# m-dayani/EORB_SLAM

Measured on AMD Instinct MI355X. Metric: front-end frames/s (event-accumulate + extract + match) per GPU; HBM GB/s vs roofline, higher is better.
Workload: dtype f32; 1 GPU; BASELINE.json configs[1]: synthetic 1000000 events/slice on 240x180 (shapes generator, DAVIS sensor pixels; raw (x,y,t,p) records resolved on the GPU through the calibrator's undistortion maps built from the EvETHZ intrinsics, as the reference loader does on the CPU), ev2im_gauss sigma=1 -> ORB-1000 (1.2, 4 levels, FAST 10/0, edge 19) -> SearchForInitialization vs previous slice; input=raw, sequences_per_gpu=1, parallelism=1 GPU

## Files before the change

eorb_slam_amd/csrc/eorb_fe.hip:

```cpp
#include "eorb_ctx.h"
#include "match_args.h"
#include "project_args.h"
#include "kfdb.h"
#include "twoview.h"
#include "sim3.h"
#include "mlpnp.h"
#include "newpts.h"
#include <stdarg.h>
#include <stdio.h>
#include <string.h>
#include <algorithm>
#include <functional>
#include <vector>

namespace eorb {

int set_err(eorb_ctx* c, int code, const char* fmt, ...)
{
    char buf[512];
    va_list ap; va_start(ap, fmt); vsnprintf(buf, sizeof(buf), fmt, ap); va_end(ap);
    if (c) c->err = buf;
    return code;
}

// ... 346 lines not shown
}

long long eorb_debug_counter(eorb_ctx* c, const char* name)
{
    if (!c || !name) return -1;
    if (!strcmp(name, "slot_calls")) return c->sl_calls;
    if (!strcmp(name, "accum_route")) return c->accum_route;
    if (!strcmp(name, "slot_rank_ok")) return c->sl_rank_ok;
    if (!strcmp(name, "dict_hits")) return c->pd_hits;
    if (!strcmp(name, "dict_misses")) return c->pd_misses;
    if (!strcmp(name, "dict_positions")) return c->pd_valid ? c->pd_K : 0;
    if (!strcmp(name, "slot_scatter_form")) return c->sl_last_rank;
    if (!strcmp(name, "slot_chunk")) return c->sl_last_chunk;
    if (!strcmp(name, "slot_binning")) return c->sl_last_binning;
    if (!strcmp(name, "kfdb_slot_cap")) return c->kfdb.slot_cap;
    if (!strcmp(name, "kfdb_word_cap")) return c->kfdb.word_cap;
    if (!strcmp(name, "slot_parts")) return c->sl_last_parts;
    if (!strcmp(name, "slot_hot_overflow")) {
        long long n = 0;
        for (int part = 0; part < std::max(c->sl_last_parts, 1); part++) {
            if (!c->sl_ws[part].hot.p) continue;
            uint32_t h = 0;
            if (hipMemcpyAsync(&h, (uint32_t*)c->sl_ws[part].hot.p + 33, sizeof(h), hipMemcpyDeviceToHost, c->stream) != hipSuccess || hipStreamSynchronize(c->stream) != hipSuccess) return -1;
            n += h;
        }
        return n;
    }
    if (!strcmp(name, "oct_lds_only")) return c->orb.oct_all_lds[0] | (c->orb.oct_all_lds[1] << 1);
    if (!strcmp(name, "oct_lds_bytes")) return c->orb.oct_lds[0];
    if (!strcmp(name, "oct_dynamic")) return c->orb.oct_dyn[0] != 0 ? 1 : 0;
    if (!strcmp(name, "oct_redo_levels")) {
        const int nl = c->orb.nlevels;
        if (!c->orb.oct_dyn[0] || !c->lvl_cnt.p || nl <= 0) return 0;
        std::vector<int32_t> f((size_t)nl);
        if (hipMemcpyAsync(f.data(), (const char*)c->lvl_cnt.p + (size_t)nl * sizeof(int32_t) + 64, sizeof(int32_t) * (size_t)nl, hipMemcpyDeviceToHost, c->stream) != hipSuccess ||
            hipStreamSynchronize(c->stream) != hipSuccess) return -1;
        long long r = 0; for (int v : f) r += v ? 1 : 0;
        return r;
    }
    if (!strcmp(name, "oct_direct_cap")) return c->orb.oct_direct_cap[0] | ((long long)c->orb.oct_direct_cap[1] << 16);
    if (!strcmp(name, "oct_scratch_bytes")) return c->orb.oct_scratch[0];
    if (!strcmp(name, "slot_hot_items")) {
        long long n = 0;
        for (int part = 0; part < std::max(c->sl_last_parts, 1); part++) {
            if (!c->sl_ws[part].hot.p) continue;
            uint32_t h[16];
// ... 3597 lines not shown
```

eorb_slam_amd/csrc/ev_plan.h:

```cpp
#pragma once
#include <math.h>
#include <stddef.h>
#include <stdint.h>
#include <algorithm>

namespace eorb {

constexpr int kTile = 8;
constexpr int kChunk = 4096;
constexpr int kScatWaves = 8;
constexpr int kSlotScatWaves = 8;
constexpr int kSlotCountWaves = 16;
constexpr int kHotCap = 8192;
constexpr int kHotRows = 240;
constexpr int kDdLog = 20;
constexpr int kDirectSlices = 8;
constexpr int64_t kDirectMaxEvents = 16384;

struct AccumShape {
    int h;
    int R, dup;
    int TX, TY, NT, NTp;
    int nbits;
    int64_t nev, per_slice;
};
inline AccumShape accum_shape(int W, int H, float sigma, int mode_count, int B, int64_t nev)
{
    AccumShape S;
    S.h = mode_count ? 0 : (int)ceil((double)sigma * 3.0);
    S.R = (2 * S.h <= kTile) ? ((S.h == 0) ? 1 : 2) : 3;
    S.dup = S.R * S.R;
    S.TX = (W + kTile - 1) / kTile; S.TY = (H + kTile - 1) / kTile; S.NT = S.TX * S.TY; S.NTp = (S.NT + 1) & ~1;
    S.nbits = 1; while ((1 << S.nbits) < S.NT) S.nbits++;
    S.nev = nev; S.per_slice = B > 0 ? nev / B : 0;
    return S;
}
// ... 135 lines not shown
inline int slot_binning_code(const SlotBinPlan& p) { return p.count | p.record << 2 | p.scatter << 4; }

inline bool plan_slot_binning(const AccumShape& S, int stride_in, int64_t nsrc, int dict, const SlotScatterChoice& sc, const AccumKnobs& K, SlotBinPlan* out)
{
    const int stride = dict ? (dict == 2 ? 2 : -4) : stride_in;
    const size_t lds_c = 4 * (((size_t)nsrc + 2) / 2) + (size_t)kSlotCountWaves * S.NTp * 2;
    const bool lds_fits = S.TX <= 127 && S.TY <= 127 && lds_c <= 159 * 1024;
    const size_t lds_p = plan_slot_lds_pre(S.NT, sc.chunk);
    const bool pre_fits = K.slot_prerank && sc.rank && lds_p <= 158 * 1024;
    const int scat = sc.rank ? kScatRank : kScatBallot;
    SlotBinPlan p{kCountLds, kRecAsIs, scat, stride, stride, lds_c, sc.lds};
    if (dict) {
        if (!lds_fits) return false;
        p.count = kCountLdsKeyed;
        if (pre_fits && dict == 2) { p.record = kRecRanked8; p.scatter = kScatPre; p.lds_scatter = lds_p; }
    }
    else if (!lds_fits) { p.count = kCountGlobal; p.lds_count = sizeof(uint32_t) * (size_t)S.NT; }
    else if (pre_fits && (stride == 16 || stride == 4 || stride == 2) && nsrc <= 65535) { p.record = kRecRanked8; p.scatter = kScatPre; p.lds_scatter = lds_p; }
    else if (stride == 16 && nsrc <= 65535 && sc.rank) { p.record = kRecShort2; p.scat_stride = 2; }
    *out = p;
    return true;
}

struct SlotGatherPlan {
    size_t lds; int wg_per_cu, nw, rounds, Gt, max_per_tile;
    uint32_t prio_ref, hot_min, hot_cap; int hot_waves;
};
inline SlotGatherPlan plan_slot_gather(const AccumShape& S, int B, int64_t nev, int nparts, int sl_null, int ncu, const AccumKnobs& K)
{
    SlotGatherPlan g;
    g.lds = (size_t)(sl_null + 1) * 256;
    g.wg_per_cu = std::max(1, (int)((160 * 1024) / g.lds));
    g.nw = std::min(16, std::max(1, 16 / g.wg_per_cu));
    if (K.slot_waves >= 1 && K.slot_waves <= 16) g.nw = K.slot_waves;
    g.nw = std::min(g.nw, std::max(1, B));
    g.rounds = K.slot_rounds >= 1 ? K.slot_rounds : 4;
    g.Gt = S.NT + g.rounds * ncu * g.wg_per_cu;
    g.max_per_tile = (B + g.nw - 1) / g.nw;
    g.prio_ref = (uint32_t)std::min<int64_t>(std::max<int64_t>(4096, nev / 2000), 0x7fffffff);
    g.hot_min = sl_null <= kHotRows ? (uint32_t)std::min<int64_t>(std::max<int64_t>(4096, nev * nparts / 16000), 0x7fffffff) : 0u;
    const long long hot_over = K.slot_hot_min;
    if (hot_over >= 0) g.hot_min = (sl_null <= kHotRows && hot_over > 0) ? (uint32_t)std::min<long long>(std::max<long long>(hot_over, 64), 0x7fffffff) : 0u;
    g.hot_cap = K.slot_hot_cap > 0 ? (uint32_t)std::min(K.slot_hot_cap, kHotCap) : (uint32_t)kHotCap;
    g.hot_waves = K.slot_hot_waves > 0 ? K.slot_hot_waves : 8 * ncu;
    return g;
}

inline int plan_first_route(const AccumShape& S, AccumRequest Q, const AccumKnobs& K, const DictState& D, int W, int H, float sigma, bool rank_ok,
                            bool slots_usable = true)
{
    SlotScatterChoice sc;
    int set = Q.raw ? kSetMaps : kSetNone, wide = 0;
    if (plan_bulk_eligible(S, Q, K) && plan_bulk_fits(S, K)) {
        if (plan_dict_usable(S, Q, K, D, W, H, sigma) && plan_slot_shape(S, Q.B, K, rank_ok, &sc)) return kFormSlots | kSetDict;
        Q.raw = 2; set = kSetPerCall;
    }
    else if (plan_direct(S, Q, K)) return kFormDirect | set;
    if (plan_slot_eligible(S, Q, K) && slots_usable && plan_slot_shape(S, Q.B, K, rank_ok, &sc)) return kFormSlots | set;
    if (Q.raw == 3 || Q.raw == 4) {
        Q.raw = 1; wide = kRouteWidened;
        if (plan_direct(S, Q, K)) return kFormDirect | set | wide;
    }
    return kFormLists | set | (plan_sparse_gather(S, Q, K) ? kRouteSparse : 0) | wide;
}

}
```

eorb_slam_amd/csrc/ev_slots.hip:

```cpp
#include "eorb_ctx.h"
#include "ev_common.h"
#include "dev_math.h"
#include "sl_hot_asm.h"
#include <algorithm>
#include <stdlib.h>
#include <string.h>
#include <vector>

namespace eorb {

constexpr uint32_t kNoSlot = 0xffu;
typedef uint16_t slot_entry;
constexpr uint32_t kEntryTag = 0x1000u;
constexpr uint16_t kNoGeo = 0xffffu;

__global__ void sl_assign_kernel(const uint32_t* __restrict__ src_info, int nsrc, int W, int H, int h, int TX,
                                 uint32_t* __restrict__ tile_nslots, uint2* __restrict__ slot_tab, uint16_t* __restrict__ slot_geo,
                                 int* __restrict__ info)
{
    const int i = blockIdx.x * blockDim.x + threadIdx.x;
    if (i >= nsrc) { if (i == nsrc) slot_geo[i] = kNoGeo; return; }
    const uint32_t w = src_info[i];
    const int xi = (int)(int16_t)(w & 0xffff), yi = (int)(int16_t)(w >> 16);
    uint2 o = make_uint2(0u, 0xffffffffu);
// ... 678 lines not shown
        const bool act = ((h >> 3) & 7u) != 0u;
        uint32_t r = 0xffffffffu;
        noise[(threadIdx.x * 33 + t) & 1023] = h;
        uint32_t rr[4];
#pragma unroll
        for (int q = 0; q < 4; q++) {
            rr[q] = 0xffffffffu;
            if (act && ((h >> (12 + q)) & 1u)) { const uint32_t o = atomicAdd(&cnt[a >> 1], 1u << (16 * (a & 1))); rr[q] = (o >> (16 * (a & 1))) & 0xffffu; }
        }
#pragma unroll
        for (int q = 0; q < 4; q++) {
            r = rr[q];
            for (int j = 0; j < 64; j++) {
                const uint32_t aj = __shfl(a, j, 64), rj = __shfl(r, j, 64);
                if (r != 0xffffffffu && rj != 0xffffffffu && j < lane && aj == a && !(rj < r)) nbad++;
            }
        }
        __syncthreads();
    }
    if (noise[threadIdx.x] == 0x12345u) nbad += 0;
    if (nbad) atomicAdd(bad, nbad);
}

constexpr int kHotBuckets = 16;
static_assert(kHotRows == SL_HOT_NROWS, "plan_slot_gather (ev_plan.h) and sl_hot_kernel's register rows");
struct HotDesc { uint32_t slice, tile, cnt, off_lo, off_hi, tx0, ty0, rows_off; };
__global__ __launch_bounds__(256) void sl_plan_kernel(const uint32_t* __restrict__ tile_cnt, const uint32_t* __restrict__ tile_base,
                                                      const int64_t* __restrict__ slice_ebase, int B, int NT, int TX, uint32_t hot_min,
                                                      const uint32_t* __restrict__ nslots, const uint32_t* __restrict__ rowbase,
                                                      uint4* __restrict__ items, uint32_t* __restrict__ tile_w, uint32_t* __restrict__ tile_m,
                                                      uint32_t* __restrict__ ctr, uint32_t* __restrict__ hot_cnt, HotDesc* __restrict__ hot_items,
                                                      uint32_t hot_cap )
{
    extern __shared__ uint32_t pc[];
    __shared__ uint32_t red[8];
    __shared__ uint32_t hb[kHotBuckets], hbase[kHotBuckets];
    uint32_t* hloc = pc + B;
    const int t = blockIdx.x, tid = threadIdx.x;
    const bool hot_ok = hot_min != 0u && nslots[t] <= (uint32_t)SL_HOT_NROWS;
    if (tid < kHotBuckets) hb[tid] = 0u;
    __syncthreads();
    for (int s = tid; s < B; s += blockDim.x) {
        const uint32_t c = tile_cnt[(size_t)s * NT + t];
        uint32_t v = c;
        if (hot_ok && c >= hot_min) {
            const int lg = 31 - __clz(c), lg0 = 31 - __clz(hot_min);
            const int q = (lg - lg0) * 4 + (int)((c >> max(lg - 2, 0)) & 3u) - (int)((hot_min >> max(lg0 - 2, 0)) & 3u);
            const int b = kHotBuckets - 1 - min(max(q, 0), kHotBuckets - 1);
            hloc[s] = ((uint32_t)b << 16) | atomicAdd(&hb[b], 1u);
            v = c | 0x80000000u;
        }
        pc[s] = v;
    }
    __syncthreads();
    if (tid < kHotBuckets) hbase[tid] = hb[tid] ? atomicAdd(&hot_cnt[tid], hb[tid]) : 0u;
    __syncthreads();
    uint32_t sum = 0, mx = 0;
    for (int s = tid; s < B; s += blockDim.x) {
        uint32_t v = pc[s];
        if (v & 0x80000000u) {
            const uint32_t c = v & 0x7fffffffu, b = hloc[s] >> 16, k = hbase[b] + (hloc[s] & 0xffffu);
            if (k < hot_cap) {
                const uint64_t off = ((uint64_t)slice_ebase[s] + tile_base[(size_t)s * NT + t]) * sizeof(slot_entry);
                HotDesc d; d.slice = (uint32_t)s; d.tile = (uint32_t)t; d.cnt = c; d.off_lo = (uint32_t)off; d.off_hi = (uint32_t)(off >> 32);
                d.tx0 = (uint32_t)(t % TX) * 8u; d.ty0 = (uint32_t)(t / TX) * 8u; d.rows_off = rowbase[t] * 256u;
                hot_items[(size_t)b * kHotCap + k] = d;
            } else { v = c; pc[s] = v; atomicAdd(&hot_cnt[33], 1u); }
        }
        if (!(v & 0x80000000u)) { sum += v; mx = max(mx, v); }
    }
    __syncthreads();
    const bool sorted = B <= 2048;
    for (int s = tid; s < B; s += blockDim.x) {
        const uint32_t c = pc[s];
        int rank = s;
        if (sorted) { rank = 0; for (int j = 0; j < B; j++) { const uint32_t v = pc[j]; rank += (v > c || (v == c && j < s)) ? 1 : 0; } }
        const uint64_t off = ((uint64_t)slice_ebase[s] + tile_base[(size_t)s * NT + t]) * sizeof(slot_entry);
        items[(size_t)t * B + rank] = make_uint4((uint32_t)s | (c & 0x80000000u), c & 0x7fffffffu, (uint32_t)off, (uint32_t)(off >> 32));
    }
#pragma unroll
    for (int d = 32; d >= 1; d >>= 1) { sum += (uint32_t)__shfl_xor((int)sum, d, 64); mx = max(mx, (uint32_t)__shfl_xor((int)mx, d, 64)); }
    if ((tid & 63) == 0) { red[tid >> 6] = sum; red[4 + (tid >> 6)] = mx; }
    __syncthreads();
    if (tid == 0) {
        tile_w[t] = red[0] + red[1] + red[2] + red[3];
        tile_m[t] = max(max(red[4], red[5]), max(red[6], red[7]));
        ctr[t] = 0u;
    }
}
__global__ __launch_bounds__(1024) void sl_tasks_kernel(const uint32_t* __restrict__ tile_w, const uint32_t* __restrict__ tile_m, int NT, int G,
                                                        int max_per_tile, uint32_t* __restrict__ scratch , uint32_t* __restrict__ task_tile, uint32_t* __restrict__ hot_cnt,
                                                        uint32_t hot_cap)
{
    if (threadIdx.x < kHotBuckets) hot_cnt[threadIdx.x] = min(hot_cnt[threadIdx.x], hot_cap);
    __shared__ unsigned long long wred[16];
    __shared__ uint32_t wsum[16], wsum2[16];
    const int tid = threadIdx.x, lane = tid & 63, wave = tid >> 6;
    unsigned long long tot = 0;
    for (int t = tid; t < NT; t += 1024) tot += tile_w[t];
#pragma unroll
    for (int d = 32; d >= 1; d >>= 1) tot += (unsigned long long)__shfl_xor((long long)tot, d, 64);
    if (lane == 0) wred[wave] = tot;
    __syncthreads();
    tot = 0;
    for (int w = 0; w < 16; w++) tot += wred[w];
    const unsigned long long spare = (unsigned long long)max(G - NT, 0);
    uint32_t* nsorted = scratch; uint32_t* tsorted = scratch + NT;
    extern __shared__ uint32_t tm[];
    for (int t = tid; t < NT; t += 1024) tm[t] = tile_m[t];
    __syncthreads();
    for (int t = tid; t < NT; t += 1024) {
        const uint32_t m = tm[t];
        int rank = 0;
        for (int u = 0; u < NT; u++) { const uint32_t v = tm[u]; rank += (v > m || (v == m && u < t)) ? 1 : 0; }
        uint32_t n = 1u + (tot ? (uint32_t)((unsigned long long)tile_w[t] * spare / tot) : 0u);
        n = min(n, (uint32_t)max(max_per_tile, 1));
        nsorted[rank] = n; tsorted[rank] = (uint32_t)t;
// ... 423 lines not shown
                                                               L.d_tile_base, p.d_entries());
        }
        else if (L.nchunks && bp.scatter == kScatRank) {
            const SlScatRankFn fn = sl_scatter_rank_fn(bp.scat_stride, waves);
            if ((rc = sl_optin(c, (const void*)fn, 159 * 1024))) return rc;
            fn<<<L.nchunks, 64 * waves, bp.lds_scatter, p.M>>>(d_ev, L.d_chunks, p.d_tab(), T.w, T.h, p.TX, p.NT, chunk, L.d_slice_eb, L.d_segbase, L.d_tile_base, p.d_entries());
        }
        else if (L.nchunks)
            sl_scatter_kernel<<<L.nchunks, 64 * kSlotScatWaves, bp.lds_scatter, p.M>>>(d_ev, L.d_chunks, p.d_tab(), bp.scat_stride, T.w, T.h, p.TX, p.TY, p.NT, chunk, L.d_slice_eb, L.d_segbase,
                                                                                         L.d_tile_base, p.d_entries());
        EORB_LAUNCH_CHECK(c, "ev_bin (slot) kernels");
    }
    EORB_HIP(c, hipEventRecord(p.E[2], p.M));
    return EORB_OK;
}

static int slots_fork_plan(const SlotPart& p)
{
    eorb_ctx* c = p.c; const BinLayout& L = p.L; const SlotGatherPlan& g = p.gp;
    EORB_HIP(c, hipEventRecord(p.E[0], p.M));
    EORB_HIP(c, hipStreamWaitEvent(p.P, p.E[0], 0));
    EORB_HIP(c, hipMemsetAsync(p.ws.hot.p, 0, 256, p.P));
    sl_plan_kernel<<<p.NT, 256, sizeof(uint32_t) * 2 * (size_t)p.B, p.P>>>(L.d_tile_cnt, L.d_tile_base, L.d_slice_eb, p.B, p.NT, p.TX, g.hot_min, p.d_nslots(), p.d_rowbase(),
                                                                             p.d_items(), p.d_tile_w(), p.d_tile_m(), p.d_ctr(), p.d_hot_cnt(), p.d_hot_items(), g.hot_cap);
    sl_tasks_kernel<<<1, 1024, sizeof(uint32_t) * (size_t)p.NT, p.P>>>(p.d_tile_w(), p.d_tile_m(), p.NT, g.Gt, g.max_per_tile, p.d_scr(), p.d_task(), p.d_hot_cnt(), g.hot_cap);
    EORB_HIP(c, hipEventRecord(p.E[1], p.P));
    return EORB_OK;
}

static int slots_gather(const SlotPart& p)
{
    eorb_ctx* c = p.c; const PosTables& T = p.T; const SlotGatherPlan& g = p.gp;
    int rc;
    SlotGather Pg{p.d_task(), p.d_items(), (const uint8_t*)p.ws.entries.p, p.d_nslots(), p.d_rowbase(), (const float*)T.sl_rows.p,
                  p.d_tile_w(), p.d_ctr(), p.d_f32, p.d_minmax_enc, p.d_info(), (int*)c->status.p, p.B, p.W, p.H, p.TX, p.NT, T.sl_null, g.prio_ref, nullptr};
#ifdef EORB_SLOT_TRACE
    EORB_HIP(c, hipMemsetAsync(c->sl_trace.p, 0, sizeof(unsigned long long) * 6 * 16 * (size_t)g.Gt + 64, p.M));
    Pg.trace = (unsigned long long*)c->sl_trace.p + 8;
    c->sl_trace_n = (long long)g.Gt * 16;
#endif
    if ((rc = sl_optin(c, (const void*)sl_gather_kernel, 160 * 1024))) return rc;
    if (g.hot_min) {
        EORB_HIP(c, hipStreamWaitEvent(p.Hs, p.E[2], 0));
        EORB_HIP(c, hipStreamWaitEvent(p.Hs, p.E[1], 0));
        sl_hot_kernel<<<g.hot_waves, 64, 0, p.Hs>>>(p.d_hot_cnt(), p.d_hot_cnt() + 32, p.d_hot_items(), kHotCap, (const float*)T.sl_rows.p, p.d_entries(), p.d_f32, p.d_minmax_enc, p.W, p.H);
    }
    EORB_HIP(c, hipEventRecord(p.E[3], p.Hs));
    if (p.G != p.M) EORB_HIP(c, hipStreamWaitEvent(p.G, p.E[2], 0));
    EORB_HIP(c, hipStreamWaitEvent(p.G, p.E[1], 0));
    {
        ProfScope ps(c, "ev_gather", p.G);
        sl_gather_kernel<<<g.Gt, 64 * g.nw, g.lds, p.G>>>(Pg);
    }
    EORB_HIP(c, hipEventRecord(p.E[4], p.G));
    EORB_LAUNCH_CHECK(c, "sl_gather_kernel");
    return EORB_OK;
}

int ev_slots_accumulate(eorb_ctx* c, const PosTables& T, const AccumShape& S, const void* d_events, int stride, const int64_t* h_offsets, int B, int W, int H,
                        float* d_f32, uint32_t* d_minmax_enc, const SlotDict* dict)
{
    const AccumKnobs K = accum_knobs(c);
    const int nparts = (K.slot_halves > 0 && B >= 2) ? 2 : 1;
    SlotScatterChoice sc;
    if (!plan_slot_shape(S, B, K, c->sl_rank_ok == 1, &sc)) return kSlotDeclined;
    for (int b = 0; b < B; b++) {
        const int64_t s = h_offsets[b], e = h_offsets[b + 1];
        if (e < s) return set_err(c, EORB_E_ARG, "ev_accumulate: offsets not monotone");
// ... 35 lines not shown
```

eorb_slam_amd/csrc/sl_hot_asm.h:

```cpp
#define SL_HOT_NROWS 240
#define SL_HOT_ASM \
    "s_setprio 3\n" \
    "v_mbcnt_lo_u32_b32 v242, -1, 0\n" \
    "v_mbcnt_hi_u32_b32 v242, -1, v242\n" \
    "v_and_b32 v249, 1, v242\n" \
    "v_lshlrev_b32 v249, 7, v249\n" \
    "v_lshlrev_b32 v252, 6, v242\n" \
    "v_and_b32 v243, 7, v242\n" \
    "v_lshrrev_b32 v244, 3, v242\n" \
    "v_lshlrev_b32 v242, 2, v242\n" \
    "v_mov_b32 v246, v243\n" \
    "v_mov_b32 v247, v244\n" \
    "s_load_dwordx16 s[36:51], %[hcnt], 0x0\n" \
    "s_waitcnt lgkmcnt(0)\n" \
    "SLH_ITEM:\n" \
    "v_mov_b32 v245, 1\n" \
    "v_mov_b32 v248, 0\n" \
    "s_mov_b64 s[62:63], exec\n" \
    "s_mov_b64 exec, 1\n" \
    "global_atomic_add v245, v248, v245, %[ticket] sc0\n" \
    "s_waitcnt vmcnt(0)\n" \
    "s_mov_b64 exec, s[62:63]\n" \
    "s_nop 0\n" \
    "v_readfirstlane_b32 s60, v245\n" \
    "s_mov_b32 s61, 0\n" \
    "s_cmp_lt_u32 s60, s36\n" \
    "s_cbranch_scc1 SLH_FOUND\n" \
    "s_sub_u32 s60, s60, s36\n" \
    "s_add_u32 s61, s61, 1\n" \
    "s_cmp_lt_u32 s60, s37\n" \
    "s_cbranch_scc1 SLH_FOUND\n" \
    "s_sub_u32 s60, s60, s37\n" \
    "s_add_u32 s61, s61, 1\n" \
    "s_cmp_lt_u32 s60, s38\n" \
    "s_cbranch_scc1 SLH_FOUND\n" \
    "s_sub_u32 s60, s60, s38\n" \
    "s_add_u32 s61, s61, 1\n" \
    "s_cmp_lt_u32 s60, s39\n" \
    "s_cbranch_scc1 SLH_FOUND\n" \
    "s_sub_u32 s60, s60, s39\n" \
    "s_add_u32 s61, s61, 1\n" \
    "s_cmp_lt_u32 s60, s40\n" \
    "s_cbranch_scc1 SLH_FOUND\n" \
    "s_sub_u32 s60, s60, s40\n" \
    "s_add_u32 s61, s61, 1\n" \
    "s_cmp_lt_u32 s60, s41\n" \
    "s_cbranch_scc1 SLH_FOUND\n" \
    "s_sub_u32 s60, s60, s41\n" \
    "s_add_u32 s61, s61, 1\n" \
    "s_cmp_lt_u32 s60, s42\n" \
    "s_cbranch_scc1 SLH_FOUND\n" \
    "s_sub_u32 s60, s60, s42\n" \
    "s_add_u32 s61, s61, 1\n" \
    "s_cmp_lt_u32 s60, s43\n" \
    "s_cbranch_scc1 SLH_FOUND\n" \
    "s_sub_u32 s60, s60, s43\n" \
    "s_add_u32 s61, s61, 1\n" \
    "s_cmp_lt_u32 s60, s44\n" \
    "s_cbranch_scc1 SLH_FOUND\n" \
    "s_sub_u32 s60, s60, s44\n" \
    "s_add_u32 s61, s61, 1\n" \
    "s_cmp_lt_u32 s60, s45\n" \
    "s_cbranch_scc1 SLH_FOUND\n" \
    "s_sub_u32 s60, s60, s45\n" \
    "s_add_u32 s61, s61, 1\n" \
    "s_cmp_lt_u32 s60, s46\n" \
    "s_cbranch_scc1 SLH_FOUND\n" \
    "s_sub_u32 s60, s60, s46\n" \
    "s_add_u32 s61, s61, 1\n" \
    "s_cmp_lt_u32 s60, s47\n" \
    "s_cbranch_scc1 SLH_FOUND\n" \
    "s_sub_u32 s60, s60, s47\n" \
    "s_add_u32 s61, s61, 1\n" \
    "s_cmp_lt_u32 s60, s48\n" \
    "s_cbranch_scc1 SLH_FOUND\n" \
    "s_sub_u32 s60, s60, s48\n" \
    "s_add_u32 s61, s61, 1\n" \
    "s_cmp_lt_u32 s60, s49\n" \
    "s_cbranch_scc1 SLH_FOUND\n" \
    "s_sub_u32 s60, s60, s49\n" \
    "s_add_u32 s61, s61, 1\n" \
    "s_cmp_lt_u32 s60, s50\n" \
    "s_cbranch_scc1 SLH_FOUND\n" \
    "s_sub_u32 s60, s60, s50\n" \
    "s_add_u32 s61, s61, 1\n" \
    "s_cmp_lt_u32 s60, s51\n" \
    "s_cbranch_scc1 SLH_FOUND\n" \
    "s_sub_u32 s60, s60, s51\n" \
    "s_add_u32 s61, s61, 1\n" \
    "s_branch SLH_DONE\n" \
    "SLH_FOUND:\n" \
    "s_mul_i32 s61, s61, %[hcap]\n" \
    "s_add_u32 s61, s61, s60\n" \
    "s_lshl_b32 s61, s61, 5\n" \
    "s_load_dwordx8 s[52:59], %[items], s61\n" \
    "s_waitcnt lgkmcnt(0)\n" \
    "s_add_u32 s64, %[rows_lo], s59\n" \
    "s_addc_u32 s65, %[rows_hi], 0\n" \
    "global_load_dword v0, v242, s[64:65] offset:0\n" \
    "global_load_dword v1, v242, s[64:65] offset:256\n" \
    "global_load_dword v2, v242, s[64:65] offset:512\n" \
    "global_load_dword v3, v242, s[64:65] offset:768\n" \
    "global_load_dword v4, v242, s[64:65] offset:1024\n" \
    "global_load_dword v5, v242, s[64:65] offset:1280\n" \
    "global_load_dword v6, v242, s[64:65] offset:1536\n" \
    "global_load_dword v7, v242, s[64:65] offset:1792\n" \
    "global_load_dword v8, v242, s[64:65] offset:2048\n" \
    "global_load_dword v9, v242, s[64:65] offset:2304\n" \
    "global_load_dword v10, v242, s[64:65] offset:2560\n" \
    "global_load_dword v11, v242, s[64:65] offset:2816\n" \
    "global_load_dword v12, v242, s[64:65] offset:3072\n" \
    "global_load_dword v13, v242, s[64:65] offset:3328\n" \
    "global_load_dword v14, v242, s[64:65] offset:3584\n" \
    "global_load_dword v15, v242, s[64:65] offset:3840\n" \
    "s_add_u32 s64, s64, 0x1000\n" \
    "s_addc_u32 s65, s65, 0\n" \
    "global_load_dword v16, v242, s[64:65] offset:0\n" \
    "global_load_dword v17, v242, s[64:65] offset:256\n" \
    "global_load_dword v18, v242, s[64:65] offset:512\n" \
// ... 226 lines not shown
    "global_load_dword v221, v242, s[64:65] offset:3328\n" \
    "global_load_dword v222, v242, s[64:65] offset:3584\n" \
    "global_load_dword v223, v242, s[64:65] offset:3840\n" \
    "s_add_u32 s64, s64, 0x1000\n" \
    "s_addc_u32 s65, s65, 0\n" \
    "global_load_dword v224, v242, s[64:65] offset:0\n" \
    "global_load_dword v225, v242, s[64:65] offset:256\n" \
    "global_load_dword v226, v242, s[64:65] offset:512\n" \
    "global_load_dword v227, v242, s[64:65] offset:768\n" \
    "global_load_dword v228, v242, s[64:65] offset:1024\n" \
    "global_load_dword v229, v242, s[64:65] offset:1280\n" \
    "global_load_dword v230, v242, s[64:65] offset:1536\n" \
    "global_load_dword v231, v242, s[64:65] offset:1792\n" \
    "global_load_dword v232, v242, s[64:65] offset:2048\n" \
    "global_load_dword v233, v242, s[64:65] offset:2304\n" \
    "global_load_dword v234, v242, s[64:65] offset:2560\n" \
    "global_load_dword v235, v242, s[64:65] offset:2816\n" \
    "global_load_dword v236, v242, s[64:65] offset:3072\n" \
    "global_load_dword v237, v242, s[64:65] offset:3328\n" \
    "global_load_dword v238, v242, s[64:65] offset:3584\n" \
    "global_load_dword v239, v242, s[64:65] offset:3840\n" \
    "s_add_u32 s64, s64, 0x1000\n" \
    "s_addc_u32 s65, s65, 0\n" \
    "v_mov_b32 v240, 0\n" \
    "v_mov_b32 v241, 0\n" \
    "s_add_u32 s100, %[ent_lo], s55\n" \
    "s_addc_u32 s101, %[ent_hi], s56\n" \
    "global_load_dword v250, v252, s[100:101]\n" \
    "v_writelane_b32 v253, s52, 0\n" \
    "v_writelane_b32 v253, s54, 1\n" \
    "v_writelane_b32 v253, s57, 2\n" \
    "v_writelane_b32 v253, s58, 3\n" \
    "s_lshr_b32 s35, s54, 6\n" \
    "s_load_dwordx16 s[36:51], s[100:101], 0x0\n" \
    "s_load_dwordx16 s[52:67], s[100:101], 0x40\n" \
    "s_mov_b32 s34, 0x80\n" \
    "s_mov_b32 s33, 0\n" \
    "s_waitcnt vmcnt(0)\n" \
    "s_set_gpr_idx_on s33, gpr_idx(SRC0)\n" \
    "SLH_LOOP:\n" \
    "v_add_u32 v251, s34, v249\n" \
    "global_load_dword v250, v251, s[100:101] offset:3968\n" \
    "s_sub_u32 s35, s35, 1\n" \
    "s_cbranch_scc1 SLH_TAIL\n" \
    "s_waitcnt lgkmcnt(0)\n" \
    "s_load_dwordx16 s[68:83], s[100:101], s34\n" \
// ... 453 lines not shown
    "s_nop 1\n" \
    "v_max_f32_dpp v248, v248, v248 row_shr:1 row_mask:0xf bank_mask:0xf bound_ctrl:0\n" \
    "s_nop 1\n" \
    "v_max_f32_dpp v248, v248, v248 row_shr:2 row_mask:0xf bank_mask:0xf bound_ctrl:0\n" \
    "s_nop 1\n" \
    "v_max_f32_dpp v248, v248, v248 row_shr:4 row_mask:0xf bank_mask:0xf bound_ctrl:0\n" \
    "s_nop 1\n" \
    "v_max_f32_dpp v248, v248, v248 row_shr:8 row_mask:0xf bank_mask:0xf bound_ctrl:0\n" \
    "s_nop 1\n" \
    "v_max_f32_dpp v248, v248, v248 row_bcast:15 row_mask:0xa bank_mask:0xf\n" \
    "s_nop 1\n" \
    "v_max_f32_dpp v248, v248, v248 row_bcast:31 row_mask:0xc bank_mask:0xf\n" \
    "s_nop 1\n" \
    "v_readlane_b32 s33, v248, 63\n" \
    "s_or_b32 s33, s33, 0x80000000\n" \
    "s_lshl_b32 s34, s52, 3\n" \
    "s_add_u32 s34, s34, 4\n" \
    "v_mov_b32 v245, s34\n" \
    "v_mov_b32 v248, s33\n" \
    "s_mov_b64 s[62:63], exec\n" \
    "s_mov_b64 exec, 1\n" \
    "global_atomic_umax v245, v248, %[mm]\n" \
    "s_mov_b64 exec, s[62:63]\n" \
    "s_load_dwordx16 s[36:51], %[hcnt], 0x0\n" \
    "s_waitcnt vmcnt(0) lgkmcnt(0)\n" \
    "s_branch SLH_ITEM\n" \
    "SLH_DONE:\n" \
    ""
#define SL_HOT_CLOBBERS "v0", "v1", "v2", "v3", "v4", "v5", "v6", "v7", "v8", "v9", "v10", "v11", "v12", "v13", "v14", "v15", "v16", "v17", "v18", "v19", "v20", "v21", "v22", "v23", "v24", "v25", "v26", "v27", "v28", "v29", "v30", "v31", "v32", "v33", "v34", "v35", "v36", "v37", "v38", "v39", "v40", "v41", "v42", "v43", "v44", "v45", "v46", "v47", "v48", "v49", "v50", "v51", "v52", "v53", "v54", "v55", "v56", "v57", "v58", "v59", "v60", "v61", "v62", "v63", "v64", "v65", "v66", "v67", "v68", "v69", "v70", "v71", "v72", "v73", "v74", "v75", "v76", "v77", "v78", "v79", "v80", "v81", "v82", "v83", "v84", "v85", "v86", "v87", "v88", "v89", "v90", "v91", "v92", "v93", "v94", "v95", "v96", "v97", "v98", "v99", "v100", "v101", "v102", "v103", "v104", "v105", "v106", "v107", "v108", "v109", "v110", "v111", "v112", "v113", "v114", "v115", "v116", "v117", "v118", "v119", "v120", "v121", "v122", "v123", "v124", "v125", "v126", "v127", "v128", "v129", "v130", "v131", "v132", "v133", "v134", "v135", "v136", "v137", "v138", "v139", "v140", "v141", "v142", "v143", "v144", "v145", "v146", "v147", "v148", "v149", "v150", "v151", "v152", "v153", "v154", "v155", "v156", "v157", "v158", "v159", "v160", "v161", "v162", "v163", "v164", "v165", "v166", "v167", "v168", "v169", "v170", "v171", "v172", "v173", "v174", "v175", "v176", "v177", "v178", "v179", "v180", "v181", "v182", "v183", "v184", "v185", "v186", "v187", "v188", "v189", "v190", "v191", "v192", "v193", "v194", "v195", "v196", "v197", "v198", "v199", "v200", "v201", "v202", "v203", "v204", "v205", "v206", "v207", "v208", "v209", "v210", "v211", "v212", "v213", "v214", "v215", "v216", "v217", "v218", "v219", "v220", "v221", "v222", "v223", "v224", "v225", "v226", "v227", "v228", "v229", "v230", "v231", "v232", "v233", "v234", "v235", "v236", "v237", "v238", "v239", "v240", "v241", "v242", "v243", "v244", "v245", "v246", "v247", "v248", "v249", "v250", "v251", "v252", "v253", "v254", "v255", "s33", "s34", "s35", "s36", "s37", "s38", "s39", "s40", "s41", "s42", "s43", "s44", "s45", "s46", "s47", "s48", "s49", "s50", "s51", "s52", "s53", "s54", "s55", "s56", "s57", "s58", "s59", "s60", "s61", "s62", "s63", "s64", "s65", "s66", "s67", "s68", "s69", "s70", "s71", "s72", "s73", "s74", "s75", "s76", "s77", "s78", "s79", "s80", "s81", "s82", "s83", "s84", "s85", "s86", "s87", "s88", "s89", "s90", "s91", "s92", "s93", "s94", "s95", "s96", "s97", "s98", "s99", "s100", "s101", "vcc", "scc", "m0", "memory"
```

Measured before the change: 47200 frames/s.

## Batch hot-tile work into runs per ticket and reuse loaded row tables

The hot-tile gather kernel now claims a run of several items per ticket instead of one, with a run length per bucket chosen on the host from the expected tile counts. Hot items are bucketed with a tunable quantization shift. Consecutive items that share the same row table skip the 240-register reload of undistortion rows. This cuts ticket atomics and redundant row loads, at the cost of coarser load balancing for big buckets and more scalar header state. A counter of row loads is added for diagnostics.

```diff
diff --git a/eorb_slam_amd/csrc/eorb_fe.hip b/eorb_slam_amd/csrc/eorb_fe.hip
--- a/eorb_slam_amd/csrc/eorb_fe.hip
+++ b/eorb_slam_amd/csrc/eorb_fe.hip
@@ -392,6 +392,16 @@
             if (!c->sl_ws[part].hot.p) continue;
             uint32_t h = 0;
             if (hipMemcpyAsync(&h, (uint32_t*)c->sl_ws[part].hot.p + 33, sizeof(h), hipMemcpyDeviceToHost, c->stream) != hipSuccess || hipStreamSynchronize(c->stream) != hipSuccess) return -1;
+            n += h;
+        }
+        return n;
+    }
+    if (!strcmp(name, "slot_hot_row_loads")) {
+        long long n = 0;
+        for (int part = 0; part < std::max(c->sl_last_parts, 1); part++) {
+            if (!c->sl_ws[part].hot.p) continue;
+            uint32_t h = 0;
+            if (hipMemcpyAsync(&h, (uint32_t*)c->sl_ws[part].hot.p + 34, sizeof(h), hipMemcpyDeviceToHost, c->stream) != hipSuccess || hipStreamSynchronize(c->stream) != hipSuccess) return -1;
             n += h;
         }
         return n;
diff --git a/eorb_slam_amd/csrc/ev_plan.h b/eorb_slam_amd/csrc/ev_plan.h
--- a/eorb_slam_amd/csrc/ev_plan.h
+++ b/eorb_slam_amd/csrc/ev_plan.h
@@ -12,6 +12,9 @@
 constexpr int kSlotScatWaves = 8;
 constexpr int kSlotCountWaves = 16;
 constexpr int kHotCap = 8192;
+constexpr int kHotBuckets = 16;
+constexpr int kHotRunRefQ = 8;
+constexpr int kHotRunLgMax = 3;
 constexpr int kHotRows = 240;
 constexpr int kDdLog = 20;
 constexpr int kDirectSlices = 8;
@@ -193,9 +196,24 @@
     return true;
 }
 
+struct HotRuns { uint8_t lg[kHotBuckets]; };
+inline
+#ifdef __HIPCC__
+__host__ __device__
+#endif
+int hot_bucket_of(uint32_t c, uint32_t hot_min, int qshift)
+{
+    int lg = 0, lg0 = 0;
+    for (uint32_t v = c; v > 1u; v >>= 1) lg++;
+    for (uint32_t v = hot_min; v > 1u; v >>= 1) lg0++;
+    const int q = (lg - lg0) * 4 + (int)((c >> (lg > 2 ? lg - 2 : 0)) & 3u) - (int)((hot_min >> (lg0 > 2 ? lg0 - 2 : 0)) & 3u);
+    const int k = (q > 0 ? q : 0) >> qshift;
+    return kHotBuckets - 1 - (k < kHotBuckets - 1 ? k : kHotBuckets - 1);
+}
 struct SlotGatherPlan {
     size_t lds; int wg_per_cu, nw, rounds, Gt, max_per_tile;
     uint32_t prio_ref, hot_min, hot_cap; int hot_waves;
+    int hot_qshift; HotRuns hot_runs;
 };
 inline SlotGatherPlan plan_slot_gather(const AccumShape& S, int B, int64_t nev, int nparts, int sl_null, int ncu, const AccumKnobs& K)
 {
@@ -214,6 +232,15 @@
     if (hot_over >= 0) g.hot_min = (sl_null <= kHotRows && hot_over > 0) ? (uint32_t)std::min<long long>(std::max<long long>(hot_over, 64), 0x7fffffff) : 0u;
     g.hot_cap = K.slot_hot_cap > 0 ? (uint32_t)std::min(K.slot_hot_cap, kHotCap) : (uint32_t)kHotCap;
     g.hot_waves = K.slot_hot_waves > 0 ? K.slot_hot_waves : 8 * ncu;
+    const int64_t top = std::max<int64_t>(nev / std::max(B, 1) / 4, 1);
+    g.hot_qshift = 0;
+    while (g.hot_qshift < 3 && ((int64_t)g.hot_min << (4 << g.hot_qshift)) < top) g.hot_qshift++;
+    for (int b = 0; b < kHotBuckets; b++) {
+        const int q_hi = ((kHotBuckets - b) << g.hot_qshift);
+        int lgr = 0;
+        while (lgr < kHotRunLgMax && (q_hi + 4 * (lgr + 1)) <= kHotRunRefQ) lgr++;
+        g.hot_runs.lg[b] = (uint8_t)lgr;
+    }
     return g;
 }
 
diff --git a/eorb_slam_amd/csrc/ev_slots.hip b/eorb_slam_amd/csrc/ev_slots.hip
--- a/eorb_slam_amd/csrc/ev_slots.hip
+++ b/eorb_slam_amd/csrc/ev_slots.hip
@@ -724,15 +724,16 @@
     if (nbad) atomicAdd(bad, nbad);
 }
 
-constexpr int kHotBuckets = 16;
 static_assert(kHotRows == SL_HOT_NROWS, "plan_slot_gather (ev_plan.h) and sl_hot_kernel's register rows");
 struct HotDesc { uint32_t slice, tile, cnt, off_lo, off_hi, tx0, ty0, rows_off; };
+constexpr int kHotRunsWord = 16, kHotTicketWord = 32, kHotOverflowWord = 33, kHotRowLoadsWord = 34, kHotLgWord = 48;
+static_assert(SL_HOT_HDR_RUNS == 4 * kHotRunsWord && SL_HOT_HDR_LG == 4 * kHotLgWord && SL_HOT_HDR_ROWLOADS == 4 * kHotRowLoadsWord, "the header as sl_hot_kernel reads it");
 __global__ __launch_bounds__(256) void sl_plan_kernel(const uint32_t* __restrict__ tile_cnt, const uint32_t* __restrict__ tile_base,
                                                       const int64_t* __restrict__ slice_ebase, int B, int NT, int TX, uint32_t hot_min,
                                                       const uint32_t* __restrict__ nslots, const uint32_t* __restrict__ rowbase,
                                                       uint4* __restrict__ items, uint32_t* __restrict__ tile_w, uint32_t* __restrict__ tile_m,
                                                       uint32_t* __restrict__ ctr, uint32_t* __restrict__ hot_cnt, HotDesc* __restrict__ hot_items,
-                                                      uint32_t hot_cap )
+                                                      uint32_t hot_cap , int hot_qshift)
 {
     extern __shared__ uint32_t pc[];
     __shared__ uint32_t red[8];
@@ -746,9 +747,7 @@
         const uint32_t c = tile_cnt[(size_t)s * NT + t];
         uint32_t v = c;
         if (hot_ok && c >= hot_min) {
-            const int lg = 31 - __clz(c), lg0 = 31 - __clz(hot_min);
-            const int q = (lg - lg0) * 4 + (int)((c >> max(lg - 2, 0)) & 3u) - (int)((hot_min >> max(lg0 - 2, 0)) & 3u);
-            const int b = kHotBuckets - 1 - min(max(q, 0), kHotBuckets - 1);
+            const int b = hot_bucket_of(c, hot_min, hot_qshift);
             hloc[s] = ((uint32_t)b << 16) | atomicAdd(&hb[b], 1u);
             v = c | 0x80000000u;
         }
@@ -767,7 +766,7 @@
                 HotDesc d; d.slice = (uint32_t)s; d.tile = (uint32_t)t; d.cnt = c; d.off_lo = (uint32_t)off; d.off_hi = (uint32_t)(off >> 32);
                 d.tx0 = (uint32_t)(t % TX) * 8u; d.ty0 = (uint32_t)(t / TX) * 8u; d.rows_off = rowbase[t] * 256u;
                 hot_items[(size_t)b * kHotCap + k] = d;
-            } else { v = c; pc[s] = v; atomicAdd(&hot_cnt[33], 1u); }
+            } else { v = c; pc[s] = v; atomicAdd(&hot_cnt[kHotOverflowWord], 1u); }
         }
         if (!(v & 0x80000000u)) { sum += v; mx = max(mx, v); }
     }
@@ -792,9 +791,14 @@
 }
 __global__ __launch_bounds__(1024) void sl_tasks_kernel(const uint32_t* __restrict__ tile_w, const uint32_t* __restrict__ tile_m, int NT, int G,
                                                         int max_per_tile, uint32_t* __restrict__ scratch , uint32_t* __restrict__ task_tile, uint32_t* __restrict__ hot_cnt,
-                                                        uint32_t hot_cap)
-{
-    if (threadIdx.x < kHotBuckets) hot_cnt[threadIdx.x] = min(hot_cnt[threadIdx.x], hot_cap);
+                                                        uint32_t hot_cap, HotRuns runs)
+{
+    if (threadIdx.x < kHotBuckets) {
+        const uint32_t n = min(hot_cnt[threadIdx.x], hot_cap), lg = runs.lg[threadIdx.x];
+        hot_cnt[threadIdx.x] = n;
+        hot_cnt[kHotRunsWord + threadIdx.x] = (n + (1u << lg) - 1u) >> lg;
+        hot_cnt[kHotLgWord + threadIdx.x] = lg;
+    }
     __shared__ unsigned long long wred[16];
     __shared__ uint32_t wsum[16], wsum2[16];
     const int tid = threadIdx.x, lane = tid & 63, wave = tid >> 6;
@@ -1264,8 +1268,8 @@
     EORB_HIP(c, hipStreamWaitEvent(p.P, p.E[0], 0));
     EORB_HIP(c, hipMemsetAsync(p.ws.hot.p, 0, 256, p.P));
     sl_plan_kernel<<<p.NT, 256, sizeof(uint32_t) * 2 * (size_t)p.B, p.P>>>(L.d_tile_cnt, L.d_tile_base, L.d_slice_eb, p.B, p.NT, p.TX, g.hot_min, p.d_nslots(), p.d_rowbase(),
-                                                                             p.d_items(), p.d_tile_w(), p.d_tile_m(), p.d_ctr(), p.d_hot_cnt(), p.d_hot_items(), g.hot_cap);
-    sl_tasks_kernel<<<1, 1024, sizeof(uint32_t) * (size_t)p.NT, p.P>>>(p.d_tile_w(), p.d_tile_m(), p.NT, g.Gt, g.max_per_tile, p.d_scr(), p.d_task(), p.d_hot_cnt(), g.hot_cap);
+                                                                             p.d_items(), p.d_tile_w(), p.d_tile_m(), p.d_ctr(), p.d_hot_cnt(), p.d_hot_items(), g.hot_cap, g.hot_qshift);
+    sl_tasks_kernel<<<1, 1024, sizeof(uint32_t) * (size_t)p.NT, p.P>>>(p.d_tile_w(), p.d_tile_m(), p.NT, g.Gt, g.max_per_tile, p.d_scr(), p.d_task(), p.d_hot_cnt(), g.hot_cap, g.hot_runs);
     EORB_HIP(c, hipEventRecord(p.E[1], p.P));
     return EORB_OK;
 }
@@ -1285,7 +1289,7 @@
     if (g.hot_min) {
         EORB_HIP(c, hipStreamWaitEvent(p.Hs, p.E[2], 0));
         EORB_HIP(c, hipStreamWaitEvent(p.Hs, p.E[1], 0));
-        sl_hot_kernel<<<g.hot_waves, 64, 0, p.Hs>>>(p.d_hot_cnt(), p.d_hot_cnt() + 32, p.d_hot_items(), kHotCap, (const float*)T.sl_rows.p, p.d_entries(), p.d_f32, p.d_minmax_enc, p.W, p.H);
+        sl_hot_kernel<<<g.hot_waves, 64, 0, p.Hs>>>(p.d_hot_cnt(), p.d_hot_cnt() + kHotTicketWord, p.d_hot_items(), kHotCap, (const float*)T.sl_rows.p, p.d_entries(), p.d_f32, p.d_minmax_enc, p.W, p.H);
     }
     EORB_HIP(c, hipEventRecord(p.E[3], p.Hs));
     if (p.G != p.M) EORB_HIP(c, hipStreamWaitEvent(p.G, p.E[2], 0));
diff --git a/eorb_slam_amd/csrc/sl_hot_asm.h b/eorb_slam_amd/csrc/sl_hot_asm.h
--- a/eorb_slam_amd/csrc/sl_hot_asm.h
+++ b/eorb_slam_amd/csrc/sl_hot_asm.h
@@ -1,4 +1,7 @@
 #define SL_HOT_NROWS 240
+#define SL_HOT_HDR_RUNS 64
+#define SL_HOT_HDR_LG 192
+#define SL_HOT_HDR_ROWLOADS 136
 #define SL_HOT_ASM \
     "s_setprio 3\n" \
     "v_mbcnt_lo_u32_b32 v242, -1, 0\n" \
@@ -11,7 +14,11 @@
     "v_lshlrev_b32 v242, 2, v242\n" \
     "v_mov_b32 v246, v243\n" \
     "v_mov_b32 v247, v244\n" \
+    "v_mov_b32 v253, -1\n" \
+    "v_writelane_b32 v253, 0, 7\n" \
     "s_load_dwordx16 s[36:51], %[hcnt], 0x0\n" \
+    "s_load_dwordx16 s[68:83], %[hcnt], 0x40\n" \
+    "s_load_dwordx16 s[84:99], %[hcnt], 0xc0\n" \
     "s_waitcnt lgkmcnt(0)\n" \
     "SLH_ITEM:\n" \
     "v_mov_b32 v245, 1\n" \
@@ -23,78 +30,157 @@
     "s_mov_b64 exec, s[62:63]\n" \
     "s_nop 0\n" \
     "v_readfirstlane_b32 s60, v245\n" \
+    "s_cmp_lt_u32 s60, s68\n" \
+    "s_cbranch_scc1 SLH_F0\n" \
+    "s_sub_u32 s60, s60, s68\n" \
+    "s_cmp_lt_u32 s60, s69\n" \
+    "s_cbranch_scc1 SLH_F1\n" \
+    "s_sub_u32 s60, s60, s69\n" \
+    "s_cmp_lt_u32 s60, s70\n" \
+    "s_cbranch_scc1 SLH_F2\n" \
+    "s_sub_u32 s60, s60, s70\n" \
+    "s_cmp_lt_u32 s60, s71\n" \
+    "s_cbranch_scc1 SLH_F3\n" \
+    "s_sub_u32 s60, s60, s71\n" \
+    "s_cmp_lt_u32 s60, s72\n" \
+    "s_cbranch_scc1 SLH_F4\n" \
+    "s_sub_u32 s60, s60, s72\n" \
+    "s_cmp_lt_u32 s60, s73\n" \
+    "s_cbranch_scc1 SLH_F5\n" \
+    "s_sub_u32 s60, s60, s73\n" \
+    "s_cmp_lt_u32 s60, s74\n" \
+    "s_cbranch_scc1 SLH_F6\n" \
+    "s_sub_u32 s60, s60, s74\n" \
+    "s_cmp_lt_u32 s60, s75\n" \
+    "s_cbranch_scc1 SLH_F7\n" \
+    "s_sub_u32 s60, s60, s75\n" \
+    "s_cmp_lt_u32 s60, s76\n" \
+    "s_cbranch_scc1 SLH_F8\n" \
+    "s_sub_u32 s60, s60, s76\n" \
+    "s_cmp_lt_u32 s60, s77\n" \
+    "s_cbranch_scc1 SLH_F9\n" \
+    "s_sub_u32 s60, s60, s77\n" \
+    "s_cmp_lt_u32 s60, s78\n" \
+    "s_cbranch_scc1 SLH_F10\n" \
+    "s_sub_u32 s60, s60, s78\n" \
+    "s_cmp_lt_u32 s60, s79\n" \
+    "s_cbranch_scc1 SLH_F11\n" \
+    "s_sub_u32 s60, s60, s79\n" \
+    "s_cmp_lt_u32 s60, s80\n" \
+    "s_cbranch_scc1 SLH_F12\n" \
+    "s_sub_u32 s60, s60, s80\n" \
+    "s_cmp_lt_u32 s60, s81\n" \
+    "s_cbranch_scc1 SLH_F13\n" \
+    "s_sub_u32 s60, s60, s81\n" \
+    "s_cmp_lt_u32 s60, s82\n" \
+    "s_cbranch_scc1 SLH_F14\n" \
+    "s_sub_u32 s60, s60, s82\n" \
+    "s_cmp_lt_u32 s60, s83\n" \
+    "s_cbranch_scc1 SLH_F15\n" \
+    "s_sub_u32 s60, s60, s83\n" \
+    "s_branch SLH_DONE\n" \
+    "SLH_F0:\n" \
     "s_mov_b32 s61, 0\n" \
-    "s_cmp_lt_u32 s60, s36\n" \
-    "s_cbranch_scc1 SLH_FOUND\n" \
-    "s_sub_u32 s60, s60, s36\n" \
-    "s_add_u32 s61, s61, 1\n" \
-    "s_cmp_lt_u32 s60, s37\n" \
-    "s_cbranch_scc1 SLH_FOUND\n" \
-    "s_sub_u32 s60, s60, s37\n" \
-    "s_add_u32 s61, s61, 1\n" \
-    "s_cmp_lt_u32 s60, s38\n" \
-    "s_cbranch_scc1 SLH_FOUND\n" \
-    "s_sub_u32 s60, s60, s38\n" \
-    "s_add_u32 s61, s61, 1\n" \
-    "s_cmp_lt_u32 s60, s39\n" \
-    "s_cbranch_scc1 SLH_FOUND\n" \
-    "s_sub_u32 s60, s60, s39\n" \
-    "s_add_u32 s61, s61, 1\n" \
-    "s_cmp_lt_u32 s60, s40\n" \
-    "s_cbranch_scc1 SLH_FOUND\n" \
-    "s_sub_u32 s60, s60, s40\n" \
-    "s_add_u32 s61, s61, 1\n" \
-    "s_cmp_lt_u32 s60, s41\n" \
-    "s_cbranch_scc1 SLH_FOUND\n" \
-    "s_sub_u32 s60, s60, s41\n" \
-    "s_add_u32 s61, s61, 1\n" \
-    "s_cmp_lt_u32 s60, s42\n" \
-    "s_cbranch_scc1 SLH_FOUND\n" \
-    "s_sub_u32 s60, s60, s42\n" \
-    "s_add_u32 s61, s61, 1\n" \
-    "s_cmp_lt_u32 s60, s43\n" \
-    "s_cbranch_scc1 SLH_FOUND\n" \
-    "s_sub_u32 s60, s60, s43\n" \
-    "s_add_u32 s61, s61, 1\n" \
-    "s_cmp_lt_u32 s60, s44\n" \
-    "s_cbranch_scc1 SLH_FOUND\n" \
-    "s_sub_u32 s60, s60, s44\n" \
-    "s_add_u32 s61, s61, 1\n" \
-    "s_cmp_lt_u32 s60, s45\n" \
-    "s_cbranch_scc1 SLH_FOUND\n" \
-    "s_sub_u32 s60, s60, s45\n" \
-    "s_add_u32 s61, s61, 1\n" \
-    "s_cmp_lt_u32 s60, s46\n" \
-    "s_cbranch_scc1 SLH_FOUND\n" \
-    "s_sub_u32 s60, s60, s46\n" \
-    "s_add_u32 s61, s61, 1\n" \
-    "s_cmp_lt_u32 s60, s47\n" \
-    "s_cbranch_scc1 SLH_FOUND\n" \
-    "s_sub_u32 s60, s60, s47\n" \
-    "s_add_u32 s61, s61, 1\n" \
-    "s_cmp_lt_u32 s60, s48\n" \
-    "s_cbranch_scc1 SLH_FOUND\n" \
-    "s_sub_u32 s60, s60, s48\n" \
-    "s_add_u32 s61, s61, 1\n" \
-    "s_cmp_lt_u32 s60, s49\n" \
-    "s_cbranch_scc1 SLH_FOUND\n" \
-    "s_sub_u32 s60, s60, s49\n" \
-    "s_add_u32 s61, s61, 1\n" \
-    "s_cmp_lt_u32 s60, s50\n" \
-    "s_cbranch_scc1 SLH_FOUND\n" \
-    "s_sub_u32 s60, s60, s50\n" \
-    "s_add_u32 s61, s61, 1\n" \
-    "s_cmp_lt_u32 s60, s51\n" \
-    "s_cbranch_scc1 SLH_FOUND\n" \
-    "s_sub_u32 s60, s60, s51\n" \
-    "s_add_u32 s61, s61, 1\n" \
-    "s_branch SLH_DONE\n" \
+    "s_mov_b32 s62, s36\n" \
+    "s_mov_b32 s63, s84\n" \
+    "s_branch SLH_FOUND\n" \
+    "SLH_F1:\n" \
+    "s_mov_b32 s61, 1\n" \
+    "s_mov_b32 s62, s37\n" \
+    "s_mov_b32 s63, s85\n" \
+    "s_branch SLH_FOUND\n" \
+    "SLH_F2:\n" \
+    "s_mov_b32 s61, 2\n" \
+    "s_mov_b32 s62, s38\n" \
+    "s_mov_b32 s63, s86\n" \
+    "s_branch SLH_FOUND\n" \
+    "SLH_F3:\n" \
+    "s_mov_b32 s61, 3\n" \
+    "s_mov_b32 s62, s39\n" \
+    "s_mov_b32 s63, s87\n" \
+    "s_branch SLH_FOUND\n" \
+    "SLH_F4:\n" \
+    "s_mov_b32 s61, 4\n" \
+    "s_mov_b32 s62, s40\n" \
+    "s_mov_b32 s63, s88\n" \
+    "s_branch SLH_FOUND\n" \
+    "SLH_F5:\n" \
+    "s_mov_b32 s61, 5\n" \
+    "s_mov_b32 s62, s41\n" \
+    "s_mov_b32 s63, s89\n" \
+    "s_branch SLH_FOUND\n" \
+    "SLH_F6:\n" \
+    "s_mov_b32 s61, 6\n" \
+    "s_mov_b32 s62, s42\n" \
+    "s_mov_b32 s63, s90\n" \
+    "s_branch SLH_FOUND\n" \
+    "SLH_F7:\n" \
+    "s_mov_b32 s61, 7\n" \
+    "s_mov_b32 s62, s43\n" \
+    "s_mov_b32 s63, s91\n" \
+    "s_branch SLH_FOUND\n" \
+    "SLH_F8:\n" \
+    "s_mov_b32 s61, 8\n" \
+    "s_mov_b32 s62, s44\n" \
+    "s_mov_b32 s63, s92\n" \
+    "s_branch SLH_FOUND\n" \
+    "SLH_F9:\n" \
+    "s_mov_b32 s61, 9\n" \
+    "s_mov_b32 s62, s45\n" \
+    "s_mov_b32 s63, s93\n" \
+    "s_branch SLH_FOUND\n" \
+    "SLH_F10:\n" \
+    "s_mov_b32 s61, 10\n" \
+    "s_mov_b32 s62, s46\n" \
+    "s_mov_b32 s63, s94\n" \
+    "s_branch SLH_FOUND\n" \
+    "SLH_F11:\n" \
+    "s_mov_b32 s61, 11\n" \
+    "s_mov_b32 s62, s47\n" \
+    "s_mov_b32 s63, s95\n" \
+    "s_branch SLH_FOUND\n" \
+    "SLH_F12:\n" \
+    "s_mov_b32 s61, 12\n" \
+    "s_mov_b32 s62, s48\n" \
+    "s_mov_b32 s63, s96\n" \
+    "s_branch SLH_FOUND\n" \
+    "SLH_F13:\n" \
+    "s_mov_b32 s61, 13\n" \
+    "s_mov_b32 s62, s49\n" \
+    "s_mov_b32 s63, s97\n" \
+    "s_branch SLH_FOUND\n" \
+    "SLH_F14:\n" \
+    "s_mov_b32 s61, 14\n" \
+    "s_mov_b32 s62, s50\n" \
+    "s_mov_b32 s63, s98\n" \
+    "s_branch SLH_FOUND\n" \
+    "SLH_F15:\n" \
+    "s_mov_b32 s61, 15\n" \
+    "s_mov_b32 s62, s51\n" \
+    "s_mov_b32 s63, s99\n" \
+    "s_branch SLH_FOUND\n" \
     "SLH_FOUND:\n" \
+    "s_lshl_b32 s60, s60, s63\n" \
+    "s_sub_u32 s62, s62, s60\n" \
+    "s_lshl_b32 s64, 1, s63\n" \
+    "s_min_u32 s62, s62, s64\n" \
+    "s_sub_u32 s62, s62, 1\n" \
     "s_mul_i32 s61, s61, %[hcap]\n" \
     "s_add_u32 s61, s61, s60\n" \
     "s_lshl_b32 s61, s61, 5\n" \
+    "SLH_LIST:\n" \
     "s_load_dwordx8 s[52:59], %[items], s61\n" \
+    "s_add_u32 s61, s61, 32\n" \
+    "v_writelane_b32 v253, s62, 5\n" \
+    "v_writelane_b32 v253, s61, 6\n" \
+    "v_readlane_b32 s33, v253, 4\n" \
     "s_waitcnt lgkmcnt(0)\n" \
+    "s_cmp_eq_u32 s33, s59\n" \
+    "s_cbranch_scc1 SLH_ROWS\n" \
+    "v_writelane_b32 v253, s59, 4\n" \
+    "v_readlane_b32 s33, v253, 7\n" \
+    "s_add_u32 s33, s33, 1\n" \
+    "v_writelane_b32 v253, s33, 7\n" \
     "s_add_u32 s64, %[rows_lo], s59\n" \
     "s_addc_u32 s65, %[rows_hi], 0\n" \
     "global_load_dword v0, v242, s[64:65] offset:0\n" \
@@ -367,6 +453,7 @@
     "global_load_dword v239, v242, s[64:65] offset:3840\n" \
     "s_add_u32 s64, s64, 0x1000\n" \
     "s_addc_u32 s65, s65, 0\n" \
+    "SLH_ROWS:\n" \
     "v_mov_b32 v240, 0\n" \
     "v_mov_b32 v241, 0\n" \
     "s_add_u32 s100, %[ent_lo], s55\n" \
@@ -866,9 +953,27 @@
     "s_mov_b64 exec, 1\n" \
     "global_atomic_umax v245, v248, %[mm]\n" \
     "s_mov_b64 exec, s[62:63]\n" \
+    "v_readlane_b32 s62, v253, 5\n" \
+    "v_readlane_b32 s61, v253, 6\n" \
+    "s_cmp_eq_u32 s62, 0\n" \
+    "s_cbranch_scc1 SLH_RUN_END\n" \
+    "s_sub_u32 s62, s62, 1\n" \
+    "s_waitcnt vmcnt(0)\n" \
+    "s_branch SLH_LIST\n" \
+    "SLH_RUN_END:\n" \
     "s_load_dwordx16 s[36:51], %[hcnt], 0x0\n" \
+    "s_load_dwordx16 s[68:83], %[hcnt], 0x40\n" \
+    "s_load_dwordx16 s[84:99], %[hcnt], 0xc0\n" \
     "s_waitcnt vmcnt(0) lgkmcnt(0)\n" \
     "s_branch SLH_ITEM\n" \
     "SLH_DONE:\n" \
+    "v_readlane_b32 s33, v253, 7\n" \
+    "v_mov_b32 v245, s33\n" \
+    "v_mov_b32 v248, 0\n" \
+    "s_mov_b64 s[62:63], exec\n" \
+    "s_mov_b64 exec, 1\n" \
+    "global_atomic_add v248, v245, %[hcnt] offset:136\n" \
+    "s_mov_b64 exec, s[62:63]\n" \
+    "s_waitcnt vmcnt(0)\n" \
     ""
 #define SL_HOT_CLOBBERS "v0", "v1", "v2", "v3", "v4", "v5", "v6", "v7", "v8", "v9", "v10", "v11", "v12", "v13", "v14", "v15", "v16", "v17", "v18", "v19", "v20", "v21", "v22", "v23", "v24", "v25", "v26", "v27", "v28", "v29", "v30", "v31", "v32", "v33", "v34", "v35", "v36", "v37", "v38", "v39", "v40", "v41", "v42", "v43", "v44", "v45", "v46", "v47", "v48", "v49", "v50", "v51", "v52", "v53", "v54", "v55", "v56", "v57", "v58", "v59", "v60", "v61", "v62", "v63", "v64", "v65", "v66", "v67", "v68", "v69", "v70", "v71", "v72", "v73", "v74", "v75", "v76", "v77", "v78", "v79", "v80", "v81", "v82", "v83", "v84", "v85", "v86", "v87", "v88", "v89", "v90", "v91", "v92", "v93", "v94", "v95", "v96", "v97", "v98", "v99", "v100", "v101", "v102", "v103", "v104", "v105", "v106", "v107", "v108", "v109", "v110", "v111", "v112", "v113", "v114", "v115", "v116", "v117", "v118", "v119", "v120", "v121", "v122", "v123", "v124", "v125", "v126", "v127", "v128", "v129", "v130", "v131", "v132", "v133", "v134", "v135", "v136", "v137", "v138", "v139", "v140", "v141", "v142", "v143", "v144", "v145", "v146", "v147", "v148", "v149", "v150", "v151", "v152", "v153", "v154", "v155", "v156", "v157", "v158", "v159", "v160", "v161", "v162", "v163", "v164", "v165", "v166", "v167", "v168", "v169", "v170", "v171", "v172", "v173", "v174", "v175", "v176", "v177", "v178", "v179", "v180", "v181", "v182", "v183", "v184", "v185", "v186", "v187", "v188", "v189", "v190", "v191", "v192", "v193", "v194", "v195", "v196", "v197", "v198", "v199", "v200", "v201", "v202", "v203", "v204", "v205", "v206", "v207", "v208", "v209", "v210", "v211", "v212", "v213", "v214", "v215", "v216", "v217", "v218", "v219", "v220", "v221", "v222", "v223", "v224", "v225", "v226", "v227", "v228", "v229", "v230", "v231", "v232", "v233", "v234", "v235", "v236", "v237", "v238", "v239", "v240", "v241", "v242", "v243", "v244", "v245", "v246", "v247", "v248", "v249", "v250", "v251", "v252", "v253", "v254", "v255", "s33", "s34", "s35", "s36", "s37", "s38", "s39", "s40", "s41", "s42", "s43", "s44", "s45", "s46", "s47", "s48", "s49", "s50", "s51", "s52", "s53", "s54", "s55", "s56", "s57", "s58", "s59", "s60", "s61", "s62", "s63", "s64", "s65", "s66", "s67", "s68", "s69", "s70", "s71", "s72", "s73", "s74", "s75", "s76", "s77", "s78", "s79", "s80", "s81", "s82", "s83", "s84", "s85", "s86", "s87", "s88", "s89", "s90", "s91", "s92", "s93", "s94", "s95", "s96", "s97", "s98", "s99", "s100", "s101", "vcc", "scc", "m0", "memory"
```

After: 47130 frames/s. About the same (-0.1%).
